# OpenGVLab/VisionLLM

Hardware: NVIDIA H100
Metric: img_text_pairs_per_sec_fwd_1024px_256tok (higher is better)
Workload: dtype bf16

## Files before the change

### visionllm_b200/csrc/attention_wgmma.cu

```cuda
#include "attention.cuh"
#include "tc_common.cuh"

namespace {

constexpr int BQ = 128, BKV = 64, THREADS = 384, CONSUMER_WARPS = 8;
template <int D> struct Cfg {
  static constexpr int NCH = D / 64;
  static constexpr int Q_BYTES = BQ * D * 2, Q_CHUNK = BQ * 128;
  static constexpr int KV_BYTES = BKV * D * 2, KV_CHUNK = BKV * 128;
  static constexpr int STG = D == 128 ? 4 : 2;
  static constexpr int SMEM = Q_BYTES + 2 * STG * KV_BYTES + 1024 + 256;
};

struct Args {
  __nv_bfloat16* o;
  long long o_bs, o_ts;
  const int* seqlens;
  int Tq, Tk, heads, kv_heads, causal;
  float scale_log2;
  const unsigned char* key_mask;
  int n_splits;
  float* ws;
};

__device__ __forceinline__ void tma_load_3d(uint32_t dst, const CUtensorMap* m, uint32_t bar, int c0, int c1, int c2) {
  asm volatile(
      "cp.async.bulk.tensor.3d.shared::cluster.global.mbarrier::complete_tx::bytes [%0], [%1, {%3, %4, %5}], [%2];" ::"r"(dst),
      "l"(reinterpret_cast<uint64_t>(m)), "r"(bar), "r"(c0), "r"(c1), "r"(c2)
      : "memory");
}
__device__ __forceinline__ uint32_t pack2(float a, float b) {
  uint32_t r;
  asm("cvt.rn.bf16x2.f32 %0, %1, %2;" : "=r"(r) : "f"(b), "f"(a));
  return r;
}
__device__ __forceinline__ float ex2(float x) {
  float y;
  asm("ex2.approx.ftz.f32 %0, %1;" : "=f"(y) : "f"(x));
  return y;
}
__device__ __forceinline__ float quad_max(float v) {
  v = fmaxf(v, __shfl_xor_sync(0xffffffffu, v, 1));
  return fmaxf(v, __shfl_xor_sync(0xffffffffu, v, 2));
}
__device__ __forceinline__ float quad_sum(float v) {
  v += __shfl_xor_sync(0xffffffffu, v, 1);
  return v + __shfl_xor_sync(0xffffffffu, v, 2);
}

template <int D, bool KM>
__global__ void __launch_bounds__(THREADS, 1)
attn_fwd_wgmma_kernel(const __grid_constant__ CUtensorMap tm_q, const __grid_constant__ CUtensorMap tm_k,
                      const __grid_constant__ CUtensorMap tm_v, const Args a) {
  constexpr int NCH = Cfg<D>::NCH, Q_BYTES = Cfg<D>::Q_BYTES, Q_CHUNK = Cfg<D>::Q_CHUNK, STG = Cfg<D>::STG;
  constexpr int KV_BYTES = Cfg<D>::KV_BYTES, KV_CHUNK = Cfg<D>::KV_CHUNK, NB = D / 128;
  extern __shared__ uint8_t smem_raw[];
  const uint32_t base = (tc::smem_u32(smem_raw) + 1023u) & ~1023u;
  const uint32_t sQ = base, sK = sQ + Q_BYTES, sV = sK + STG * KV_BYTES, bar = sV + STG * KV_BYTES;
  const uint32_t q_full = bar;
  auto k_full = [&](int s) { return bar + 8 * (1 + s); };
  auto v_full = [&](int s) { return bar + 8 * (1 + STG + s); };
  auto k_empty = [&](int s) { return bar + 8 * (1 + 2 * STG + s); };
  auto v_empty = [&](int s) { return bar + 8 * (1 + 3 * STG + s); };

  const int warp = threadIdx.x >> 5, lane = threadIdx.x & 31;
  const int split = blockIdx.x % a.n_splits;
  const int q0 = (blockIdx.x / a.n_splits) * BQ, head = blockIdx.y, b = blockIdx.z;
  const int kvh = head / (a.heads / a.kv_heads);
  const int len = a.seqlens ? min(a.seqlens[b], a.Tk) : a.Tk;
  const int coff = a.Tk - a.Tq;
  int k_end = len;
  if (a.causal) k_end = min(k_end, q0 + BQ + coff);
  const int n_all = k_end > 0 ? (k_end + BKV - 1) / BKV : 0;
  const int per_split = (n_all + a.n_splits - 1) / a.n_splits;
  const int t0 = split * per_split;
  const int n = max(0, min(n_all - t0, per_split));

  if (warp == 0 && lane == 0) { tc::tma_prefetch_desc(&tm_q); tc::tma_prefetch_desc(&tm_k); tc::tma_prefetch_desc(&tm_v); }
  if (warp == 1 && lane == 0) {
    tc::mbar_init(q_full, 1);
    for (int s = 0; s < STG; ++s) {
      tc::mbar_init(k_full(s), 1); tc::mbar_init(v_full(s), 1);
      tc::mbar_init(k_empty(s), CONSUMER_WARPS); tc::mbar_init(v_empty(s), CONSUMER_WARPS);
    }
    tc::mbar_fence_init();
  }
  __syncthreads();

  if (warp < 4) {
    tc::reg_dealloc<40>();
    if (warp == 0 && tc::elect_one() && n > 0) {
      tc::mbar_arrive_expect_tx(q_full, Q_BYTES);
      for (int h = 0; h < NCH; ++h) tma_load_3d(sQ + h * Q_CHUNK, &tm_q, q_full, head * D + h * 64, q0, b);
      for (int j = 0; j < n; ++j) {
        const int s = j % STG;
        const uint32_t ph = ((j / STG) & 1) ^ 1;
        tc::mbar_wait(k_empty(s), ph);
        tc::mbar_arrive_expect_tx(k_full(s), KV_BYTES);
        for (int h = 0; h < NCH; ++h) tma_load_3d(sK + s * KV_BYTES + h * KV_CHUNK, &tm_k, k_full(s), kvh * D + h * 64, (t0 + j) * BKV, b);
        tc::mbar_wait(v_empty(s), ph);
        tc::mbar_arrive_expect_tx(v_full(s), KV_BYTES);
        for (int h = 0; h < NCH; ++h) tma_load_3d(sV + s * KV_BYTES + h * KV_CHUNK, &tm_v, v_full(s), kvh * D + h * 64, (t0 + j) * BKV, b);
      }
    }
    return;
  }

  tc::reg_alloc<232>();
  const int wg = (warp - 4) >> 2;
  const int r0 = q0 + wg * 64 + (warp & 3) * 16 + (lane >> 2), r1 = r0 + 8;
  const int cq = 2 * (lane & 3);
  const uint32_t sQw = sQ + wg * 64 * 128;
  float o[NB][64];
#pragma unroll
  for (int nb = 0; nb < NB; ++nb)
#pragma unroll
    for (int i = 0; i < 64; ++i) o[nb][i] = 0.f;
  float m0 = -INFINITY, m1 = -INFINITY, l0 = 0.f, l1 = 0.f;
  if (n > 0) tc::mbar_wait(q_full, 0);
  for (int j = 0; j < n; ++j) {
    const int s = j % STG;
    const uint32_t ph = (j / STG) & 1;
    float sc[32];
    tc::mbar_wait(k_full(s), ph);
    tc::wgmma_fence();
#pragma unroll
    for (int kk = 0; kk < D / 16; ++kk)
      tc::wgmma_m64n64k16_ss(sc, tc::wgmma_desc_sw128(sQw + (kk >> 2) * Q_CHUNK + (kk & 3) * 32, 16, 1024),
                             tc::wgmma_desc_sw128(sK + s * KV_BYTES + (kk >> 2) * KV_CHUNK + (kk & 3) * 32, 16, 1024), kk != 0);
    tc::wgmma_commit();
    tc::wgmma_wait<0>();
    tc::acc_fence(sc);
    if (lane == 0) tc::mbar_arrive(k_empty(s));
    const int n0 = (t0 + j) * BKV;
    if constexpr (KM) {
      const unsigned char* km = a.key_mask + (size_t)b * a.Tk + n0;
#pragma unroll
      for (int jb = 0; jb < 8; ++jb)
#pragma unroll
        for (int e = 0; e < 2; ++e) {
          const int c = 8 * jb + cq + e;
          if (n0 + c < a.Tk && !__ldg(km + c)) { sc[4 * jb + e] = -INFINITY; sc[4 * jb + 2 + e] = -INFINITY; }
        }
    }
    if ((n0 + BKV > len) || (a.causal && (n0 + BKV - 1 > q0 + coff))) {
      const int lim0 = (a.causal ? min(len, r0 + coff + 1) : len) - n0;
      const int lim1 = (a.causal ? min(len, r1 + coff + 1) : len) - n0;
#pragma unroll
      for (int jb = 0; jb < 8; ++jb)
#pragma unroll
        for (int e = 0; e < 2; ++e) {
          const int c = 8 * jb + cq + e;
          if (c >= lim0) sc[4 * jb + e] = -INFINITY;
          if (c >= lim1) sc[4 * jb + 2 + e] = -INFINITY;
        }
    }
    float mx0 = -INFINITY, mx1 = -INFINITY;
#pragma unroll
    for (int jb = 0; jb < 8; ++jb) {
      mx0 = fmaxf(mx0, fmaxf(sc[4 * jb], sc[4 * jb + 1]));
      mx1 = fmaxf(mx1, fmaxf(sc[4 * jb + 2], sc[4 * jb + 3]));
    }
    const float mn0 = fmaxf(m0, quad_max(mx0) * a.scale_log2), mn1 = fmaxf(m1, quad_max(mx1) * a.scale_log2);
    const float corr0 = (m0 == -INFINITY) ? 0.f : ex2(m0 - mn0), corr1 = (m1 == -INFINITY) ? 0.f : ex2(m1 - mn1);
    m0 = mn0; m1 = mn1;
    const float mu0 = (m0 == -INFINITY) ? 0.f : m0, mu1 = (m1 == -INFINITY) ? 0.f : m1;
    float rs0 = 0.f, rs1 = 0.f;
    uint32_t p[4][4];
#pragma unroll
    for (int jb = 0; jb < 8; ++jb) {
      const float p00 = ex2(fmaf(sc[4 * jb], a.scale_log2, -mu0)), p01 = ex2(fmaf(sc[4 * jb + 1], a.scale_log2, -mu0));
      const float p10 = ex2(fmaf(sc[4 * jb + 2], a.scale_log2, -mu1)), p11 = ex2(fmaf(sc[4 * jb + 3], a.scale_log2, -mu1));
      rs0 += p00 + p01; rs1 += p10 + p11;
      p[jb >> 1][(jb & 1) * 2] = pack2(p00, p01);
      p[jb >> 1][(jb & 1) * 2 + 1] = pack2(p10, p11);
    }
    l0 = l0 * corr0 + rs0; l1 = l1 * corr1 + rs1;
#pragma unroll
    for (int nb = 0; nb < NB; ++nb)
#pragma unroll
      for (int i = 0; i < 64; i += 4) {
        o[nb][i] *= corr0; o[nb][i + 1] *= corr0; o[nb][i + 2] *= corr1; o[nb][i + 3] *= corr1;
      }
    tc::mbar_wait(v_full(s), ph);
#pragma unroll
    for (int nb = 0; nb < NB; ++nb) tc::acc_fence(o[nb]);
    tc::wgmma_fence();
#pragma unroll
    for (int kk = 0; kk < BKV / 16; ++kk)
#pragma unroll
      for (int nb = 0; nb < NB; ++nb)
        tc::wgmma_m64n128k16_rs(o[nb], p[kk], tc::wgmma_desc_sw128(sV + s * KV_BYTES + kk * 2048 + nb * 2 * KV_CHUNK, KV_CHUNK, 1024), 1);
    tc::wgmma_commit();
    tc::wgmma_wait<0>();
#pragma unroll
    for (int nb = 0; nb < NB; ++nb) tc::acc_fence(o[nb]);
    if (lane == 0) tc::mbar_arrive(v_empty(s));
  }
  l0 = quad_sum(l0); l1 = quad_sum(l1);

  if (a.n_splits > 1) {
    float* w0 = a.ws + ((((size_t)b * a.heads + head) * a.n_splits + split) * a.Tq + r0) * (D + 2);
    float* w1 = w0 + (size_t)8 * (D + 2);
#pragma unroll
    for (int nb = 0; nb < NB; ++nb)
#pragma unroll
      for (int jb = 0; jb < 16; ++jb) {
        const int c = nb * 128 + 8 * jb + cq;
        if (r0 < a.Tq) *reinterpret_cast<float2*>(w0 + c) = make_float2(o[nb][4 * jb], o[nb][4 * jb + 1]);
        if (r1 < a.Tq) *reinterpret_cast<float2*>(w1 + c) = make_float2(o[nb][4 * jb + 2], o[nb][4 * jb + 3]);
      }
    if (cq == 0) {
      if (r0 < a.Tq) { w0[D] = m0; w0[D + 1] = l0; }
      if (r1 < a.Tq) { w1[D] = m1; w1[D + 1] = l1; }
    }
    return;
  }
  const float inv0 = l0 > 0.f ? 1.f / l0 : 0.f, inv1 = l1 > 0.f ? 1.f / l1 : 0.f;
  __nv_bfloat16* op0 = a.o + b * a.o_bs + (long long)r0 * a.o_ts + head * D;
  __nv_bfloat16* op1 = op0 + 8 * a.o_ts;
#pragma unroll
  for (int nb = 0; nb < NB; ++nb)
#pragma unroll
    for (int jb = 0; jb < 16; ++jb) {
      const int c = nb * 128 + 8 * jb + cq;
      if (r0 < a.Tq) *reinterpret_cast<uint32_t*>(op0 + c) = pack2(o[nb][4 * jb] * inv0, o[nb][4 * jb + 1] * inv0);
      if (r1 < a.Tq) *reinterpret_cast<uint32_t*>(op1 + c) = pack2(o[nb][4 * jb + 2] * inv1, o[nb][4 * jb + 3] * inv1);
    }
}

int make_tmap(CUtensorMap* m, const void* base, uint64_t cols, uint64_t tokens, uint64_t batch, uint64_t token_pitch,
              uint64_t batch_pitch, uint32_t box_rows) {
  PFN_cuTensorMapEncodeTiled_v12000 enc = vllm_tma_encoder();
  if (!enc) return -100;
  cuuint64_t dims[3] = {cols, tokens, batch};
  cuuint64_t strides[2] = {token_pitch * 2, batch_pitch * 2};
  cuuint32_t box[3] = {64, box_rows, 1};
  cuuint32_t estr[3] = {1, 1, 1};
  if (batch == 1) strides[1] = token_pitch * 2 * (tokens > 0 ? tokens : 1);
  CUresult r = enc(m, CU_TENSOR_MAP_DATA_TYPE_BFLOAT16, 3, const_cast<void*>(base), dims, strides, box, estr,
                   CU_TENSOR_MAP_INTERLEAVE_NONE, CU_TENSOR_MAP_SWIZZLE_128B, CU_TENSOR_MAP_L2_PROMOTION_L2_256B,
                   CU_TENSOR_MAP_FLOAT_OOB_FILL_NONE);
  return r == CUDA_SUCCESS ? 0 : -101;
}

}

template <int D, bool KM>
static int launch_wgmma(const CUtensorMap& tq, const CUtensorMap& tk, const CUtensorMap& tv, const Args& a, int batch,
                        cudaStream_t st) {
  auto kern = attn_fwd_wgmma_kernel<D, KM>;
  const cudaError_t e = vllm_smem_optin(kern, Cfg<D>::SMEM);
  if (e != cudaSuccess) return (int)e;
  dim3 grid((unsigned)(((a.Tq + BQ - 1) / BQ) * a.n_splits), a.heads, batch);
  kern<<<grid, THREADS, Cfg<D>::SMEM, st>>>(tq, tk, tv, a);
  VLLM_CHECK_LAUNCH();
  return VLLM_OK;
}

int vllm_attention_wgmma(const AttnArgs& at, int batch, int head_dim, cudaStream_t st) {
  if (head_dim != 128 && head_dim != 256) return VLLM_EUNSUPPORTED;
  const uint64_t D = (uint64_t)head_dim;
  CUtensorMap tq, tk, tv;
  if (make_tmap(&tq, at.q, (uint64_t)at.heads * D, at.Tq, batch, at.q_ts, at.q_bs, BQ)) return VLLM_EUNSUPPORTED;
  if (make_tmap(&tk, at.k, (uint64_t)at.kv_heads * D, at.Tk, batch, at.k_ts, at.k_bs, BKV)) return VLLM_EUNSUPPORTED;
  if (make_tmap(&tv, at.v, (uint64_t)at.kv_heads * D, at.Tk, batch, at.v_ts, at.v_bs, BKV)) return VLLM_EUNSUPPORTED;
  Args a;
  a.o = at.o; a.o_bs = at.o_bs; a.o_ts = at.o_ts; a.seqlens = at.seqlens; a.Tq = at.Tq; a.Tk = at.Tk;
  a.heads = at.heads; a.kv_heads = at.kv_heads; a.causal = at.causal; a.scale_log2 = at.scale_log2;
  a.key_mask = at.key_mask; a.n_splits = at.n_splits; a.ws = at.ws;
  if (head_dim == 128) return at.key_mask ? launch_wgmma<128, true>(tq, tk, tv, a, batch, st) : launch_wgmma<128, false>(tq, tk, tv, a, batch, st);
  return at.key_mask ? launch_wgmma<256, true>(tq, tk, tv, a, batch, st) : launch_wgmma<256, false>(tq, tk, tv, a, batch, st);
}
```

### visionllm_b200/csrc/tc_common.cuh

```cuda
#pragma once
#include <cuda.h>
#include <cuda_runtime.h>
#include <stdint.h>

namespace tc {

__device__ __forceinline__ uint32_t smem_u32(const void* p) {
  return static_cast<uint32_t>(__cvta_generic_to_shared(p));
}
__device__ __forceinline__ bool elect_one() {
  uint32_t pred = 0;
  asm volatile(
      "{\n\t.reg .pred P;\n\telect.sync _|P, 0xffffffff;\n\tselp.u32 %0, 1, 0, P;\n\t}\n"
      : "=r"(pred));
  return pred != 0;
}

__device__ __forceinline__ void mbar_init(uint32_t bar, uint32_t count) {
  asm volatile("mbarrier.init.shared::cta.b64 [%0], %1;" ::"r"(bar), "r"(count) : "memory");
}
__device__ __forceinline__ void mbar_fence_init() {
  asm volatile("fence.mbarrier_init.release.cluster;" ::: "memory");
}
__device__ __forceinline__ void mbar_arrive_expect_tx(uint32_t bar, uint32_t bytes) {
  asm volatile("mbarrier.arrive.expect_tx.shared::cta.b64 _, [%0], %1;" ::"r"(bar), "r"(bytes) : "memory");
}
__device__ __forceinline__ void mbar_arrive(uint32_t bar) {
  asm volatile("mbarrier.arrive.shared::cta.b64 _, [%0];" ::"r"(bar) : "memory");
}
__device__ __forceinline__ bool mbar_try_wait(uint32_t bar, uint32_t parity) {
  uint32_t ok;
  asm volatile(
      "{\n\t.reg .pred p;\n\tmbarrier.try_wait.parity.shared::cta.b64 p, [%1], %2;\n\tselp.u32 %0, 1, 0, p;\n\t}\n"
      : "=r"(ok)
      : "r"(bar), "r"(parity)
      : "memory");
  return ok != 0;
}
__device__ __forceinline__ void mbar_wait(uint32_t bar, uint32_t parity) {
  while (!mbar_try_wait(bar, parity)) {
  }
}
__device__ __forceinline__ void tma_prefetch_desc(const CUtensorMap* m) {
  asm volatile("prefetch.tensormap [%0];" ::"l"(reinterpret_cast<uint64_t>(m)) : "memory");
}
__device__ __forceinline__ void tma_load_2d(uint32_t dst, const CUtensorMap* m, uint32_t bar, int c0, int c1) {
  asm volatile(
      "cp.async.bulk.tensor.2d.shared::cluster.global.mbarrier::complete_tx::bytes [%0], [%1, {%3, %4}], [%2];" ::"r"(dst),
      "l"(reinterpret_cast<uint64_t>(m)), "r"(bar), "r"(c0), "r"(c1)
      : "memory");
}
__device__ __forceinline__ void tma_store_2d(const CUtensorMap* m, uint32_t src, int c0, int c1) {
  asm volatile("cp.async.bulk.tensor.2d.global.shared::cta.bulk_group [%0, {%2, %3}], [%1];" ::"l"(reinterpret_cast<uint64_t>(m)),
               "r"(src), "r"(c0), "r"(c1)
               : "memory");
}
__device__ __forceinline__ void bulk_commit() { asm volatile("cp.async.bulk.commit_group;" ::: "memory"); }
template <int N> __device__ __forceinline__ void bulk_wait_read() { asm volatile("cp.async.bulk.wait_group.read %0;" ::"n"(N) : "memory"); }
template <int N> __device__ __forceinline__ void bulk_wait() { asm volatile("cp.async.bulk.wait_group %0;" ::"n"(N) : "memory"); }
__device__ __forceinline__ void fence_proxy_async_smem() { asm volatile("fence.proxy.async.shared::cta;" ::: "memory"); }

__device__ __forceinline__ void cp_async_vec_word(uint32_t dst, const void* v, long long len, long long b0, int i) {
  const uintptr_t base = reinterpret_cast<uintptr_t>(v);
  const uintptr_t w = ((base + b0) & ~uintptr_t(3)) + 4u * i;
  const long long left = (long long)(base + len) - (long long)w;
  const int n = left >= 4 ? 4 : left > 0 ? (int)left : 0;
  asm volatile("cp.async.ca.shared.global [%0], [%1], 4, %2;" ::"r"(dst + 4u * i), "l"(w), "r"(n) : "memory");
}
__device__ __forceinline__ void cp_async_wait_all() { asm volatile("cp.async.wait_all;" ::: "memory"); }

template <int N> __device__ __forceinline__ void reg_dealloc() { asm volatile("setmaxnreg.dec.sync.aligned.u32 %0;" ::"n"(N)); }
template <int N> __device__ __forceinline__ void reg_alloc() { asm volatile("setmaxnreg.inc.sync.aligned.u32 %0;" ::"n"(N)); }
__device__ __forceinline__ void named_bar_sync(int id, int threads) {
  asm volatile("bar.sync %0, %1;" ::"r"(id), "r"(threads) : "memory");
}

__device__ __forceinline__ void wgmma_fence() { asm volatile("wgmma.fence.sync.aligned;" ::: "memory"); }
__device__ __forceinline__ void wgmma_commit() { asm volatile("wgmma.commit_group.sync.aligned;" ::: "memory"); }
template <int N> __device__ __forceinline__ void wgmma_wait() { asm volatile("wgmma.wait_group.sync.aligned %0;" ::"n"(N) : "memory"); }
template <int N> __device__ __forceinline__ void acc_fence(float (&d)[N]) {
#pragma unroll
  for (int i = 0; i < N; ++i) asm volatile("" : "+f"(d[i])::"memory");
}

template <int TA, int TB>
__device__ __forceinline__ void wgmma_m64n128k16_ss(float (&d)[64], uint64_t adesc, uint64_t bdesc, uint32_t accumulate) {
  asm volatile(
      "{\n\t.reg .pred p;\n\tsetp.ne.b32 p, %66, 0;\n\t"
      "wgmma.mma_async.sync.aligned.m64n128k16.f32.bf16.bf16 {"
      "%0, %1, %2, %3, %4, %5, %6, %7, %8, %9, %10, %11, %12, %13, %14, %15, %16, %17, %18, %19, %20, %21, "
      "%22, %23, %24, %25, %26, %27, %28, %29, %30, %31, %32, %33, %34, %35, %36, %37, %38, %39, %40, %41, "
      "%42, %43, %44, %45, %46, %47, %48, %49, %50, %51, %52, %53, %54, %55, %56, %57, %58, %59, %60, %61, "
      "%62, %63 "
      "}, %64, %65, p, 1, 1, %67, %68;\n\t}\n"
      : "+f"(d[0]), "+f"(d[1]), "+f"(d[2]), "+f"(d[3]), "+f"(d[4]), "+f"(d[5]), "+f"(d[6]), "+f"(d[7]),
        "+f"(d[8]), "+f"(d[9]), "+f"(d[10]), "+f"(d[11]), "+f"(d[12]), "+f"(d[13]), "+f"(d[14]), "+f"(d[15]),
        "+f"(d[16]), "+f"(d[17]), "+f"(d[18]), "+f"(d[19]), "+f"(d[20]), "+f"(d[21]), "+f"(d[22]), "+f"(d[23]),
        "+f"(d[24]), "+f"(d[25]), "+f"(d[26]), "+f"(d[27]), "+f"(d[28]), "+f"(d[29]), "+f"(d[30]), "+f"(d[31]),
        "+f"(d[32]), "+f"(d[33]), "+f"(d[34]), "+f"(d[35]), "+f"(d[36]), "+f"(d[37]), "+f"(d[38]), "+f"(d[39]),
        "+f"(d[40]), "+f"(d[41]), "+f"(d[42]), "+f"(d[43]), "+f"(d[44]), "+f"(d[45]), "+f"(d[46]), "+f"(d[47]),
        "+f"(d[48]), "+f"(d[49]), "+f"(d[50]), "+f"(d[51]), "+f"(d[52]), "+f"(d[53]), "+f"(d[54]), "+f"(d[55]),
        "+f"(d[56]), "+f"(d[57]), "+f"(d[58]), "+f"(d[59]), "+f"(d[60]), "+f"(d[61]), "+f"(d[62]), "+f"(d[63])
      : "l"(adesc), "l"(bdesc), "r"(accumulate), "n"(TA), "n"(TB));
}
template <int TA, int TB>
__device__ __forceinline__ void wgmma_m64n256k16_ss(float (&d)[128], uint64_t adesc, uint64_t bdesc, uint32_t accumulate) {
  asm volatile(
      "{\n\t.reg .pred p;\n\tsetp.ne.b32 p, %130, 0;\n\t"
      "wgmma.mma_async.sync.aligned.m64n256k16.f32.bf16.bf16 {"
      "%0, %1, %2, %3, %4, %5, %6, %7, %8, %9, %10, %11, %12, %13, %14, %15, %16, %17, %18, %19, %20, %21, "
      "%22, %23, %24, %25, %26, %27, %28, %29, %30, %31, %32, %33, %34, %35, %36, %37, %38, %39, %40, %41, %42, %43, "
      "%44, %45, %46, %47, %48, %49, %50, %51, %52, %53, %54, %55, %56, %57, %58, %59, %60, %61, %62, %63, %64, %65, "
      "%66, %67, %68, %69, %70, %71, %72, %73, %74, %75, %76, %77, %78, %79, %80, %81, %82, %83, %84, %85, %86, %87, "
      "%88, %89, %90, %91, %92, %93, %94, %95, %96, %97, %98, %99, %100, %101, %102, %103, %104, %105, %106, %107, %108, %109, "
      "%110, %111, %112, %113, %114, %115, %116, %117, %118, %119, %120, %121, %122, %123, %124, %125, %126, %127 "
      "}, %128, %129, p, 1, 1, %131, %132;\n\t}\n"
      : "+f"(d[0]), "+f"(d[1]), "+f"(d[2]), "+f"(d[3]), "+f"(d[4]), "+f"(d[5]), "+f"(d[6]), "+f"(d[7]),
        "+f"(d[8]), "+f"(d[9]), "+f"(d[10]), "+f"(d[11]), "+f"(d[12]), "+f"(d[13]), "+f"(d[14]), "+f"(d[15]),
        "+f"(d[16]), "+f"(d[17]), "+f"(d[18]), "+f"(d[19]), "+f"(d[20]), "+f"(d[21]), "+f"(d[22]), "+f"(d[23]),
        "+f"(d[24]), "+f"(d[25]), "+f"(d[26]), "+f"(d[27]), "+f"(d[28]), "+f"(d[29]), "+f"(d[30]), "+f"(d[31]),
        "+f"(d[32]), "+f"(d[33]), "+f"(d[34]), "+f"(d[35]), "+f"(d[36]), "+f"(d[37]), "+f"(d[38]), "+f"(d[39]),
        "+f"(d[40]), "+f"(d[41]), "+f"(d[42]), "+f"(d[43]), "+f"(d[44]), "+f"(d[45]), "+f"(d[46]), "+f"(d[47]),
        "+f"(d[48]), "+f"(d[49]), "+f"(d[50]), "+f"(d[51]), "+f"(d[52]), "+f"(d[53]), "+f"(d[54]), "+f"(d[55]),
        "+f"(d[56]), "+f"(d[57]), "+f"(d[58]), "+f"(d[59]), "+f"(d[60]), "+f"(d[61]), "+f"(d[62]), "+f"(d[63]),
        "+f"(d[64]), "+f"(d[65]), "+f"(d[66]), "+f"(d[67]), "+f"(d[68]), "+f"(d[69]), "+f"(d[70]), "+f"(d[71]),
        "+f"(d[72]), "+f"(d[73]), "+f"(d[74]), "+f"(d[75]), "+f"(d[76]), "+f"(d[77]), "+f"(d[78]), "+f"(d[79]),
        "+f"(d[80]), "+f"(d[81]), "+f"(d[82]), "+f"(d[83]), "+f"(d[84]), "+f"(d[85]), "+f"(d[86]), "+f"(d[87]),
        "+f"(d[88]), "+f"(d[89]), "+f"(d[90]), "+f"(d[91]), "+f"(d[92]), "+f"(d[93]), "+f"(d[94]), "+f"(d[95]),
        "+f"(d[96]), "+f"(d[97]), "+f"(d[98]), "+f"(d[99]), "+f"(d[100]), "+f"(d[101]), "+f"(d[102]), "+f"(d[103]),
        "+f"(d[104]), "+f"(d[105]), "+f"(d[106]), "+f"(d[107]), "+f"(d[108]), "+f"(d[109]), "+f"(d[110]), "+f"(d[111]),
        "+f"(d[112]), "+f"(d[113]), "+f"(d[114]), "+f"(d[115]), "+f"(d[116]), "+f"(d[117]), "+f"(d[118]), "+f"(d[119]),
        "+f"(d[120]), "+f"(d[121]), "+f"(d[122]), "+f"(d[123]), "+f"(d[124]), "+f"(d[125]), "+f"(d[126]), "+f"(d[127])
      : "l"(adesc), "l"(bdesc), "r"(accumulate), "n"(TA), "n"(TB));
}
__device__ __forceinline__ void wgmma_m64n64k16_ss(float (&d)[32], uint64_t adesc, uint64_t bdesc, uint32_t accumulate) {
  asm volatile(
      "{\n\t.reg .pred p;\n\tsetp.ne.b32 p, %34, 0;\n\t"
      "wgmma.mma_async.sync.aligned.m64n64k16.f32.bf16.bf16 {"
      "%0, %1, %2, %3, %4, %5, %6, %7, %8, %9, %10, %11, %12, %13, %14, %15, %16, %17, %18, %19, %20, %21, "
      "%22, %23, %24, %25, %26, %27, %28, %29, %30, %31 "
      "}, %32, %33, p, 1, 1, 0, 0;\n\t}\n"
      : "+f"(d[0]), "+f"(d[1]), "+f"(d[2]), "+f"(d[3]), "+f"(d[4]), "+f"(d[5]), "+f"(d[6]), "+f"(d[7]),
        "+f"(d[8]), "+f"(d[9]), "+f"(d[10]), "+f"(d[11]), "+f"(d[12]), "+f"(d[13]), "+f"(d[14]), "+f"(d[15]),
        "+f"(d[16]), "+f"(d[17]), "+f"(d[18]), "+f"(d[19]), "+f"(d[20]), "+f"(d[21]), "+f"(d[22]), "+f"(d[23]),
        "+f"(d[24]), "+f"(d[25]), "+f"(d[26]), "+f"(d[27]), "+f"(d[28]), "+f"(d[29]), "+f"(d[30]), "+f"(d[31])
      : "l"(adesc), "l"(bdesc), "r"(accumulate));
}
__device__ __forceinline__ void wgmma_m64n128k16_rs(float (&d)[64], const uint32_t (&a)[4], uint64_t bdesc, uint32_t accumulate) {
  asm volatile(
      "{\n\t.reg .pred p;\n\tsetp.ne.b32 p, %69, 0;\n\t"
      "wgmma.mma_async.sync.aligned.m64n128k16.f32.bf16.bf16 {"
      "%0, %1, %2, %3, %4, %5, %6, %7, %8, %9, %10, %11, %12, %13, %14, %15, %16, %17, %18, %19, %20, %21, "
      "%22, %23, %24, %25, %26, %27, %28, %29, %30, %31, %32, %33, %34, %35, %36, %37, %38, %39, %40, %41, "
      "%42, %43, %44, %45, %46, %47, %48, %49, %50, %51, %52, %53, %54, %55, %56, %57, %58, %59, %60, %61, "
      "%62, %63 "
      "}, {%64, %65, %66, %67}, %68, p, 1, 1, 1;\n\t}\n"
      : "+f"(d[0]), "+f"(d[1]), "+f"(d[2]), "+f"(d[3]), "+f"(d[4]), "+f"(d[5]), "+f"(d[6]), "+f"(d[7]),
        "+f"(d[8]), "+f"(d[9]), "+f"(d[10]), "+f"(d[11]), "+f"(d[12]), "+f"(d[13]), "+f"(d[14]), "+f"(d[15]),
        "+f"(d[16]), "+f"(d[17]), "+f"(d[18]), "+f"(d[19]), "+f"(d[20]), "+f"(d[21]), "+f"(d[22]), "+f"(d[23]),
        "+f"(d[24]), "+f"(d[25]), "+f"(d[26]), "+f"(d[27]), "+f"(d[28]), "+f"(d[29]), "+f"(d[30]), "+f"(d[31]),
        "+f"(d[32]), "+f"(d[33]), "+f"(d[34]), "+f"(d[35]), "+f"(d[36]), "+f"(d[37]), "+f"(d[38]), "+f"(d[39]),
        "+f"(d[40]), "+f"(d[41]), "+f"(d[42]), "+f"(d[43]), "+f"(d[44]), "+f"(d[45]), "+f"(d[46]), "+f"(d[47]),
        "+f"(d[48]), "+f"(d[49]), "+f"(d[50]), "+f"(d[51]), "+f"(d[52]), "+f"(d[53]), "+f"(d[54]), "+f"(d[55]),
        "+f"(d[56]), "+f"(d[57]), "+f"(d[58]), "+f"(d[59]), "+f"(d[60]), "+f"(d[61]), "+f"(d[62]), "+f"(d[63])
      : "r"(a[0]), "r"(a[1]), "r"(a[2]), "r"(a[3]), "l"(bdesc), "r"(accumulate));
}

__device__ __forceinline__ uint64_t wgmma_desc_sw128(uint32_t smem_addr, uint32_t lbo_bytes, uint32_t sbo_bytes) {
  uint64_t d = 0;
  d |= (uint64_t)((smem_addr & 0x3FFFF) >> 4);
  d |= (uint64_t)(lbo_bytes >> 4) << 16;
  d |= (uint64_t)(sbo_bytes >> 4) << 32;
  d |= (uint64_t)1 << 62;
  return d;
}

}

#include <cudaTypedefs.h>
static inline PFN_cuTensorMapEncodeTiled_v12000 vllm_tma_encoder() {
  static PFN_cuTensorMapEncodeTiled_v12000 fn = nullptr;
  if (!fn) {
    void* p = nullptr;
    cudaDriverEntryPointQueryResult q;
    if (cudaGetDriverEntryPoint("cuTensorMapEncodeTiled", &p, cudaEnableDefault, &q) == cudaSuccess &&
        q == cudaDriverEntryPointSuccess)
      fn = reinterpret_cast<PFN_cuTensorMapEncodeTiled_v12000>(p);
  }
  return fn;
}
static inline int vllm_make_tmap_2d(CUtensorMap* m, const void* base, uint64_t rows, uint64_t cols, uint64_t ld,
                                    uint32_t box_rows, bool f32 = false) {
  PFN_cuTensorMapEncodeTiled_v12000 enc = vllm_tma_encoder();
  if (!enc) return -100;
  const uint32_t elt = f32 ? 4 : 2;
  cuuint64_t dims[2] = {cols, rows};
  cuuint64_t strides[1] = {ld * elt};
  cuuint32_t box[2] = {128 / elt, box_rows};
  cuuint32_t estr[2] = {1, 1};
  CUresult r = enc(m, f32 ? CU_TENSOR_MAP_DATA_TYPE_FLOAT32 : CU_TENSOR_MAP_DATA_TYPE_BFLOAT16, 2, const_cast<void*>(base),
                   dims, strides, box, estr, CU_TENSOR_MAP_INTERLEAVE_NONE, CU_TENSOR_MAP_SWIZZLE_128B,
                   CU_TENSOR_MAP_L2_PROMOTION_L2_256B, CU_TENSOR_MAP_FLOAT_OOB_FILL_NONE);
  return r == CUDA_SUCCESS ? 0 : -101;
}
```

Before: 6.947.

## Overlap QK^T of next tile with PV and softmax in wgmma attention

Restructures the consumer loop into a software pipeline: the S=QK^T wgmma for tile j+1 is issued before the PV wgmma for tile j, and softmax runs while PV is in flight (wait<1>). For D=128, Q is held in registers via ldmatrix and fed to a new register-source m64n64k16 wgmma. Key-mask loading is replaced with a warp ballot, and consumer warpgroups past the end of Tq exit early, with barrier counts adjusted to match. This raises register pressure and depends on the ldmatrix swizzle math matching the TMA layout.

```diff
diff --git a/visionllm_b200/csrc/attention_wgmma.cu b/visionllm_b200/csrc/attention_wgmma.cu
--- a/visionllm_b200/csrc/attention_wgmma.cu
+++ b/visionllm_b200/csrc/attention_wgmma.cu
@@ -3,7 +3,7 @@
 
 namespace {
 
-constexpr int BQ = 128, BKV = 64, THREADS = 384, CONSUMER_WARPS = 8;
+constexpr int BQ = 128, BKV = 64, THREADS = 384;
 template <int D> struct Cfg {
   static constexpr int NCH = D / 64;
   static constexpr int Q_BYTES = BQ * D * 2, Q_CHUNK = BQ * 128;
@@ -38,6 +38,10 @@
   float y;
   asm("ex2.approx.ftz.f32 %0, %1;" : "=f"(y) : "f"(x));
   return y;
+}
+__device__ __forceinline__ void ldmatrix_x4(uint32_t (&r)[4], uint32_t addr) {
+  asm volatile("ldmatrix.sync.aligned.m8n8.x4.shared.b16 {%0, %1, %2, %3}, [%4];"
+               : "=r"(r[0]), "=r"(r[1]), "=r"(r[2]), "=r"(r[3]) : "r"(addr));
 }
 __device__ __forceinline__ float quad_max(float v) {
   v = fmaxf(v, __shfl_xor_sync(0xffffffffu, v, 1));
@@ -75,13 +79,14 @@
   const int per_split = (n_all + a.n_splits - 1) / a.n_splits;
   const int t0 = split * per_split;
   const int n = max(0, min(n_all - t0, per_split));
+  const int live_wg = min(2, (a.Tq - q0 + 63) / 64);
 
   if (warp == 0 && lane == 0) { tc::tma_prefetch_desc(&tm_q); tc::tma_prefetch_desc(&tm_k); tc::tma_prefetch_desc(&tm_v); }
   if (warp == 1 && lane == 0) {
     tc::mbar_init(q_full, 1);
     for (int s = 0; s < STG; ++s) {
       tc::mbar_init(k_full(s), 1); tc::mbar_init(v_full(s), 1);
-      tc::mbar_init(k_empty(s), CONSUMER_WARPS); tc::mbar_init(v_empty(s), CONSUMER_WARPS);
+      tc::mbar_init(k_empty(s), 4 * live_wg); tc::mbar_init(v_empty(s), 4 * live_wg);
     }
     tc::mbar_fence_init();
   }
@@ -106,8 +111,9 @@
     return;
   }
 
+  const int wg = (warp - 4) >> 2;
+  if (wg >= live_wg) return;
   tc::reg_alloc<232>();
-  const int wg = (warp - 4) >> 2;
   const int r0 = q0 + wg * 64 + (warp & 3) * 16 + (lane >> 2), r1 = r0 + 8;
   const int cq = 2 * (lane & 3);
   const uint32_t sQw = sQ + wg * 64 * 128;
@@ -117,31 +123,48 @@
 #pragma unroll
     for (int i = 0; i < 64; ++i) o[nb][i] = 0.f;
   float m0 = -INFINITY, m1 = -INFINITY, l0 = 0.f, l1 = 0.f;
-  if (n > 0) tc::mbar_wait(q_full, 0);
-  for (int j = 0; j < n; ++j) {
+  float corr0 = 0.f, corr1 = 0.f;
+  float sc[32];
+  constexpr int QREG = D == 128 ? D / 16 : 1;
+  uint32_t qa[QREG][4];
+  auto load_q = [&] {
+    if constexpr (D == 128) {
+      const int row = wg * 64 + (warp & 3) * 16 + (lane & 15);
+#pragma unroll
+      for (int kk = 0; kk < QREG; ++kk) {
+        const int unit = (kk & 3) * 2 + (lane >> 4);
+        ldmatrix_x4(qa[kk], sQ + (kk >> 2) * Q_CHUNK + row * 128 + ((unit ^ (row & 7)) << 4));
+      }
+    }
+  };
+  auto issue_s = [&](int j) {
     const int s = j % STG;
-    const uint32_t ph = (j / STG) & 1;
-    float sc[32];
-    tc::mbar_wait(k_full(s), ph);
+    tc::mbar_wait(k_full(s), (j / STG) & 1);
     tc::wgmma_fence();
 #pragma unroll
-    for (int kk = 0; kk < D / 16; ++kk)
-      tc::wgmma_m64n64k16_ss(sc, tc::wgmma_desc_sw128(sQw + (kk >> 2) * Q_CHUNK + (kk & 3) * 32, 16, 1024),
-                             tc::wgmma_desc_sw128(sK + s * KV_BYTES + (kk >> 2) * KV_CHUNK + (kk & 3) * 32, 16, 1024), kk != 0);
+    for (int kk = 0; kk < D / 16; ++kk) {
+      const uint64_t kdesc = tc::wgmma_desc_sw128(sK + s * KV_BYTES + (kk >> 2) * KV_CHUNK + (kk & 3) * 32, 16, 1024);
+      if constexpr (D == 128)
+        tc::wgmma_m64n64k16_rs(sc, qa[kk], kdesc, kk != 0);
+      else
+        tc::wgmma_m64n64k16_ss(sc, tc::wgmma_desc_sw128(sQw + (kk >> 2) * Q_CHUNK + (kk & 3) * 32, 16, 1024), kdesc, kk != 0);
+    }
     tc::wgmma_commit();
-    tc::wgmma_wait<0>();
+  };
+  auto softmax = [&](int j) {
     tc::acc_fence(sc);
-    if (lane == 0) tc::mbar_arrive(k_empty(s));
+    if (lane == 0) tc::mbar_arrive(k_empty(j % STG));
     const int n0 = (t0 + j) * BKV;
     if constexpr (KM) {
-      const unsigned char* km = a.key_mask + (size_t)b * a.Tk + n0;
+      const unsigned char* km = a.key_mask + (size_t)b * a.Tk + n0 + 2 * lane;
+      const int c = n0 + 2 * lane;
+      const uint32_t kb0 = __ballot_sync(0xffffffffu, c >= a.Tk || __ldg(km)) >> (lane & 3);
+      const uint32_t kb1 = __ballot_sync(0xffffffffu, c + 1 >= a.Tk || __ldg(km + 1)) >> (lane & 3);
 #pragma unroll
       for (int jb = 0; jb < 8; ++jb)
 #pragma unroll
-        for (int e = 0; e < 2; ++e) {
-          const int c = 8 * jb + cq + e;
-          if (n0 + c < a.Tk && !__ldg(km + c)) { sc[4 * jb + e] = -INFINITY; sc[4 * jb + 2 + e] = -INFINITY; }
-        }
+        for (int e = 0; e < 2; ++e)
+          if (!(((e ? kb1 : kb0) >> (4 * jb)) & 1u)) { sc[4 * jb + e] = -INFINITY; sc[4 * jb + 2 + e] = -INFINITY; }
     }
     if ((n0 + BKV > len) || (a.causal && (n0 + BKV - 1 > q0 + coff))) {
       const int lim0 = (a.causal ? min(len, r0 + coff + 1) : len) - n0;
@@ -162,27 +185,34 @@
       mx1 = fmaxf(mx1, fmaxf(sc[4 * jb + 2], sc[4 * jb + 3]));
     }
     const float mn0 = fmaxf(m0, quad_max(mx0) * a.scale_log2), mn1 = fmaxf(m1, quad_max(mx1) * a.scale_log2);
-    const float corr0 = (m0 == -INFINITY) ? 0.f : ex2(m0 - mn0), corr1 = (m1 == -INFINITY) ? 0.f : ex2(m1 - mn1);
+    corr0 = (m0 == -INFINITY) ? 0.f : ex2(m0 - mn0); corr1 = (m1 == -INFINITY) ? 0.f : ex2(m1 - mn1);
     m0 = mn0; m1 = mn1;
     const float mu0 = (m0 == -INFINITY) ? 0.f : m0, mu1 = (m1 == -INFINITY) ? 0.f : m1;
     float rs0 = 0.f, rs1 = 0.f;
-    uint32_t p[4][4];
 #pragma unroll
     for (int jb = 0; jb < 8; ++jb) {
-      const float p00 = ex2(fmaf(sc[4 * jb], a.scale_log2, -mu0)), p01 = ex2(fmaf(sc[4 * jb + 1], a.scale_log2, -mu0));
-      const float p10 = ex2(fmaf(sc[4 * jb + 2], a.scale_log2, -mu1)), p11 = ex2(fmaf(sc[4 * jb + 3], a.scale_log2, -mu1));
-      rs0 += p00 + p01; rs1 += p10 + p11;
-      p[jb >> 1][(jb & 1) * 2] = pack2(p00, p01);
-      p[jb >> 1][(jb & 1) * 2 + 1] = pack2(p10, p11);
+      sc[4 * jb] = ex2(fmaf(sc[4 * jb], a.scale_log2, -mu0)); sc[4 * jb + 1] = ex2(fmaf(sc[4 * jb + 1], a.scale_log2, -mu0));
+      sc[4 * jb + 2] = ex2(fmaf(sc[4 * jb + 2], a.scale_log2, -mu1)); sc[4 * jb + 3] = ex2(fmaf(sc[4 * jb + 3], a.scale_log2, -mu1));
+      rs0 += sc[4 * jb] + sc[4 * jb + 1]; rs1 += sc[4 * jb + 2] + sc[4 * jb + 3];
     }
     l0 = l0 * corr0 + rs0; l1 = l1 * corr1 + rs1;
+  };
+  auto pack = [&](uint32_t (&p)[4][4]) {
+#pragma unroll
+    for (int jb = 0; jb < 8; ++jb) {
+      p[jb >> 1][(jb & 1) * 2] = pack2(sc[4 * jb], sc[4 * jb + 1]);
+      p[jb >> 1][(jb & 1) * 2 + 1] = pack2(sc[4 * jb + 2], sc[4 * jb + 3]);
+    }
+  };
+  auto issue_pv = [&](int j, const uint32_t (&p)[4][4]) {
+    const int s = j % STG;
 #pragma unroll
     for (int nb = 0; nb < NB; ++nb)
 #pragma unroll
       for (int i = 0; i < 64; i += 4) {
         o[nb][i] *= corr0; o[nb][i + 1] *= corr0; o[nb][i + 2] *= corr1; o[nb][i + 3] *= corr1;
       }
-    tc::mbar_wait(v_full(s), ph);
+    tc::mbar_wait(v_full(s), (j / STG) & 1);
 #pragma unroll
     for (int nb = 0; nb < NB; ++nb) tc::acc_fence(o[nb]);
     tc::wgmma_fence();
@@ -192,10 +222,34 @@
       for (int nb = 0; nb < NB; ++nb)
         tc::wgmma_m64n128k16_rs(o[nb], p[kk], tc::wgmma_desc_sw128(sV + s * KV_BYTES + kk * 2048 + nb * 2 * KV_CHUNK, KV_CHUNK, 1024), 1);
     tc::wgmma_commit();
+  };
+  auto retire_pv = [&](int j) {
     tc::wgmma_wait<0>();
 #pragma unroll
     for (int nb = 0; nb < NB; ++nb) tc::acc_fence(o[nb]);
-    if (lane == 0) tc::mbar_arrive(v_empty(s));
+    if (lane == 0) tc::mbar_arrive(v_empty(j % STG));
+  };
+  if (n > 0) {
+    tc::mbar_wait(q_full, 0);
+    load_q();
+    issue_s(0);
+    tc::wgmma_wait<0>();
+    softmax(0);
+  }
+  for (int j = 0; j + 1 < n; ++j) {
+    uint32_t p[4][4];
+    pack(p);
+    issue_s(j + 1);
+    issue_pv(j, p);
+    tc::wgmma_wait<1>();
+    softmax(j + 1);
+    retire_pv(j);
+  }
+  if (n > 0) {
+    uint32_t p[4][4];
+    pack(p);
+    issue_pv(n - 1, p);
+    retire_pv(n - 1);
   }
   l0 = quad_sum(l0); l1 = quad_sum(l1);
 
diff --git a/visionllm_b200/csrc/tc_common.cuh b/visionllm_b200/csrc/tc_common.cuh
--- a/visionllm_b200/csrc/tc_common.cuh
+++ b/visionllm_b200/csrc/tc_common.cuh
@@ -146,6 +146,19 @@
         "+f"(d[24]), "+f"(d[25]), "+f"(d[26]), "+f"(d[27]), "+f"(d[28]), "+f"(d[29]), "+f"(d[30]), "+f"(d[31])
       : "l"(adesc), "l"(bdesc), "r"(accumulate));
 }
+__device__ __forceinline__ void wgmma_m64n64k16_rs(float (&d)[32], const uint32_t (&a)[4], uint64_t bdesc, uint32_t accumulate) {
+  asm volatile(
+      "{\n\t.reg .pred p;\n\tsetp.ne.b32 p, %37, 0;\n\t"
+      "wgmma.mma_async.sync.aligned.m64n64k16.f32.bf16.bf16 {"
+      "%0, %1, %2, %3, %4, %5, %6, %7, %8, %9, %10, %11, %12, %13, %14, %15, %16, %17, %18, %19, %20, %21, "
+      "%22, %23, %24, %25, %26, %27, %28, %29, %30, %31 "
+      "}, {%32, %33, %34, %35}, %36, p, 1, 1, 0;\n\t}\n"
+      : "+f"(d[0]), "+f"(d[1]), "+f"(d[2]), "+f"(d[3]), "+f"(d[4]), "+f"(d[5]), "+f"(d[6]), "+f"(d[7]),
+        "+f"(d[8]), "+f"(d[9]), "+f"(d[10]), "+f"(d[11]), "+f"(d[12]), "+f"(d[13]), "+f"(d[14]), "+f"(d[15]),
+        "+f"(d[16]), "+f"(d[17]), "+f"(d[18]), "+f"(d[19]), "+f"(d[20]), "+f"(d[21]), "+f"(d[22]), "+f"(d[23]),
+        "+f"(d[24]), "+f"(d[25]), "+f"(d[26]), "+f"(d[27]), "+f"(d[28]), "+f"(d[29]), "+f"(d[30]), "+f"(d[31])
+      : "r"(a[0]), "r"(a[1]), "r"(a[2]), "r"(a[3]), "l"(bdesc), "r"(accumulate));
+}
 __device__ __forceinline__ void wgmma_m64n128k16_rs(float (&d)[64], const uint32_t (&a)[4], uint64_t bdesc, uint32_t accumulate) {
   asm volatile(
       "{\n\t.reg .pred p;\n\tsetp.ne.b32 p, %69, 0;\n\t"
```

After: 6.993, median of 6. About the same (+0.7%).
